# xiph/vorbis

Measured on NVIDIA H100. Metric: stereo_blocks_per_sec_mdct_psy, higher is better.
Workload: dtype f32

## Files before the change

### include/vorbis_b200.h

```cpp
#ifndef VORBIS_B200_H
#define VORBIS_B200_H

#include <stddef.h>
#include <stdint.h>

#ifdef __cplusplus
extern "C" {
#endif

#define VB200_OK        0
#define VB200_EFAULT  (-129)
#define VB200_EIMPL   (-130)
#define VB200_EINVAL  (-131)

#define VB200_P_BANDS        17
#define VB200_P_LEVELS        8
#define VB200_P_NOISECURVES   3
#define VB200_EHMER_MAX      56
#define VB200_COMPAND_LEVELS 40
#define VB200_PACKETBLOBS    15
#define VB200_MAX_CHANNELS  255
#define VB200_VE_BANDS        7
#define VB200_MAX_COUPLING  256

// ... 68 lines not shown
  float   stretch_penalty;
  float   preecho_minenergy;
  vb200_residue_setup residue[2][VB200_MAX_SUBMAPS];
} vb200_setup;

typedef struct vb200_block_desc {
  int32_t lW;
  int32_t nW;
  int32_t blocktype;
  float   ampmax;
} vb200_block_desc;

typedef struct vb200_ctx vb200_ctx;

int  vb200_ctx_create(const vb200_setup *setup, int device, vb200_ctx **out);
void vb200_ctx_destroy(vb200_ctx *ctx);
int  vb200_device_count(void);
const char *vb200_last_error(void);
int  vb200_ctx_table(vb200_ctx *ctx, int W, int which, void *dst, int cap);
uint64_t vb200_launch_count(vb200_ctx *ctx);
int  vb200_set_profiling(vb200_ctx *ctx, int on);
int  vb200_phaseA_kernel_ms(vb200_ctx *ctx, float *ms3);
int  vb200_encode_dsp_kernel_ms(vb200_ctx *ctx, float *ms6);
int  vb200_debug_phase_cycles(vb200_ctx *ctx, unsigned long long *out16, int reset);

int vb200_mdct_forward_dev (vb200_ctx*, int W, int nvec, const float *d_in, float *d_out, void *stream);
int vb200_mdct_forward     (vb200_ctx*, int W, int nvec, const float *in,   float *out);
int vb200_mdct_backward_dev(vb200_ctx*, int W, int nvec, const float *d_in, float *d_out, void *stream);
int vb200_mdct_backward    (vb200_ctx*, int W, int nvec, const float *in,   float *out);
int vb200_apply_window     (vb200_ctx*, int W, int nvec, const int32_t *lW, const int32_t *nW, float *data);
int vb200_drft_forward     (vb200_ctx*, int W, int nvec, float *data);

int vb200_noisemask        (vb200_ctx*, int look, int nvec, const float *logmdct, float *noise);
int vb200_tonemask         (vb200_ctx*, int look, int nvec, const float *logfft,
                            const float *global_specmax, const float *local_specmax, float *tone);
int vb200_offset_and_mix   (vb200_ctx*, int look, int nvec, int offset_select,
                            const float *noise, const float *tone,
                            float *mdct, const float *logmdct, float *logmask);

typedef struct vb200_phaseA_io {
  const float *pcm;
  const vb200_block_desc *desc;
  float *mdct;
  float *logmdct;
  float *logmask;
  float *ampmax_out;
  float *tap_noise;
// ... 303 lines not shown
```

### vorbis_b200/csrc/vb200.cu

```cuda
#include <cuda_runtime.h>
#include <algorithm>
#include <atomic>
#include <cstdio>
#include <cstdlib>
#include <cstring>
#include <mutex>
#include <string>
#include <type_traits>
#include <vector>

#include "vorbis_b200.h"
#include "vb200_tables.h"
#include "vb200_kernels.cuh"
#include "vb200_cqn.cuh"
#include "vb200_psy3.cuh"
#include "vb200_floor1.cuh"
#include "vb200_env.cuh"
#include "vb200_res.cuh"
#include "vb200_streams.cuh"
#include "vb200_managed.cuh"
#include "vb200_entropy_enc.cuh"
#include "vb200_bitrate.cuh"
#include "floor1_db_table.h"

// ... 405 lines not shown
  const void *src = nullptr; size_t cnt = 0, el = 4;
  switch (which) {
    case 0: src = h.trig.data(); cnt = h.trig.size(); break;
    case 1: src = h.bitrev.data(); cnt = h.bitrev.size(); break;
    case 2: src = h.win.data(); cnt = h.win.size(); break;
    case 3: src = h.wa.data(); cnt = h.wa.size(); break;
    default: return VB200_EINVAL;
  }
  if ((size_t)cap < cnt) return VB200_EINVAL;
  memcpy(dst, src, cnt * el);
  return (int)cnt;
}

extern "C" uint64_t vb200_launch_count(vb200_ctx *c) { return c ? c->launches.load() : 0; }

extern "C" int vb200_set_profiling(vb200_ctx *c, int on) {
  if (!c) return fail(VB200_EINVAL, "null context");
  CU(cudaSetDevice(c->device));
  if (on) for (auto &e : c->ev) if (!e) CU(cudaEventCreate(&e));
  c->profiling = on != 0;
  return 0;
}

extern "C" int vb200_debug_phase_cycles(vb200_ctx *c, unsigned long long *out16, int reset) {
  if (!c || !out16) return fail(VB200_EINVAL, "null argument");
  CU(cudaSetDevice(c->device));
  void *p; int rc;
  if ((rc = ensure_buf(c->cycles, 16 * sizeof(unsigned long long), &p))) return rc;
  CU(cudaDeviceSynchronize());
  CU(cudaMemcpy(out16, p, 16 * sizeof(unsigned long long), cudaMemcpyDeviceToHost));
  if (reset) CU(cudaMemset(p, 0, 16 * sizeof(unsigned long long)));
  return 0;
}

extern "C" int vb200_phaseA_kernel_ms(vb200_ctx *c, float *ms3) {
  if (!c || !ms3 || !c->ev[0]) return fail(VB200_EINVAL, "profiling not enabled");
  CU(cudaSetDevice(c->device));
  CU(cudaEventSynchronize(c->ev[3]));
  for (int i = 0; i < 3; i++) CU(cudaEventElapsedTime(ms3 + i, c->ev[i], c->ev[i + 1]));
  return 0;
}

extern "C" int vb200_encode_dsp_kernel_ms(vb200_ctx *c, float *ms6) {
  if (!c || !ms6 || !c->ev[0]) return fail(VB200_EINVAL, "profiling not enabled");
  CU(cudaSetDevice(c->device));
  CU(cudaEventSynchronize(c->ev[6]));
  for (int i = 0; i < 6; i++) CU(cudaEventElapsedTime(ms6 + i, c->ev[i], c->ev[i + 1]));
  return 0;
}


template <int NC>
__global__ void __launch_bounds__(256)
k_mdct_forward(XformDev X, int nvec, const float *__restrict__ in, float *__restrict__ out) {
  extern __shared__ __align__(16) float sm[];
  const int N = NC ? NC : X.N, tid = threadIdx.x, nt = blockDim.x;
  float *sx[2] = {sm, sm + N};
  float *sw = sm + 2 * N, *pad = sm + 3 * N;
  auto stage = [&](float *dst, int v) {
    const float *src = in + (size_t)v * N;
    const unsigned d = smem_u32(dst);
    for (int i = tid; i < (N >> 2); i += nt) cp_async16(d + 16u * (unsigned)i, src + 4 * i);
    cp_async_commit();
  };
  int v = blockIdx.x, buf = 0;
  if (v < nvec) stage(sx[0], v);
  for (; v < nvec; v += gridDim.x, buf ^= 1) {
    cp_async_wait_all();
    __syncthreads();
    if (v + (int)gridDim.x < nvec) stage(sx[buf ^ 1], v + gridDim.x);
    dev_mdct_forward<NC>(X, sx[buf], sw, out + (size_t)v * (N >> 1), tid, nt, pad);
    __syncthreads();
  }
}

template <int NC>
__global__ void __launch_bounds__(256)
k_mdct_backward(XformDev X, int nvec, const float *__restrict__ in, float *__restrict__ out) {
  extern __shared__ __align__(16) float sm[];
  const int N = NC ? NC : X.N, n2 = N >> 1, tid = threadIdx.x, nt = blockDim.x;
  float *sin_ = sm, *so = sm + n2;
  for (int v = blockIdx.x; v < nvec; v += gridDim.x) {
    const float4 *src = reinterpret_cast<const float4 *>(in + (size_t)v * n2);
    for (int i = tid; i < (n2 >> 2); i += nt) reinterpret_cast<float4 *>(sin_)[i] = __ldg(src + i);
    __syncthreads();
    dev_mdct_backward<NC>(X, sin_, so, tid, nt);
    float4 *dst = reinterpret_cast<float4 *>(out + (size_t)v * N);
    for (int i = tid; i < (N >> 2); i += nt) dst[i] = reinterpret_cast<float4 *>(so)[i];
    __syncthreads();
  }
}

__global__ void __launch_bounds__(256)
k_apply_window(WinDev Wd, int W, int nvec, const int *__restrict__ lW, const int *__restrict__ nW,
// ... 30 lines not shown
  const void *base;
  int fmt;
  int bps, hop;
  long long stride;
  const int2 *blk_src;
};

__device__ __forceinline__ void blk_origin(const PcmSrc &src, int blk, long long &st, long long &off) {
  if (src.blk_src) { const int2 o = __ldg(src.blk_src + blk); st = o.x; off = o.y; }
  else { const int s = blk / src.bps; st = s; off = (long long)(blk - s * src.bps) * src.hop; }
}

__device__ __forceinline__ float *mdct_pad_buffer(float *sf) {
#ifdef VB200_NO_FLY_PAD
  (void)sf; return nullptr;
#else
  return sf;
#endif
}

#ifndef XF_MINB
#define XF_MINB 5
#endif
template <int NC>
__global__ void __launch_bounds__(256, XF_MINB)
k_phaseA_transform(XformDev X, WinDev Wd, int W, int ch, int nrows,
                   PcmSrc src, const vb200_block_desc *__restrict__ desc,
                   float *__restrict__ mdct, float *__restrict__ logfft, float *__restrict__ lmax) {
  extern __shared__ __align__(16) float sm[];
  __shared__ float s_red[8];
  const int N = NC ? NC : X.N, n = N >> 1, tid = threadIdx.x, nt = blockDim.x;
  float *sx = sm, *sw = sm + fft_buf_floats(N), *sf = sw + N;
  const float scale = 4.f / (float)N;
  const float scale_dB = add345(todB_dev(scale));
  float *sraw = sf + fft_buf_floats(N);
  auto stage = [&](int r) -> int {
    const int b2 = r / ch, c = r - b2 * ch;
    const char *g = nullptr;
    int mode = 0;
    if (src.fmt == VB200_PCM_S16_INTERLEAVED) {
      long long st, off; blk_origin(src, b2, st, off);
      g = reinterpret_cast<const char *>(reinterpret_cast<const short *>(src.base) + (st * src.stride + off) * ch);
      mode = ch == 2 ? 2 : 0;
    } else {
      const float *pf = reinterpret_cast<const float *>(src.base);
      if (src.fmt == VB200_PCM_F32_PLANAR) {
        long long st, off; blk_origin(src, b2, st, off);
        pf += (st * ch + c) * src.stride + off;
      } else {
        pf += (size_t)r * N;
      }
      g = reinterpret_cast<const char *>(pf);
// ... 30 lines not shown
      const short *p16 = reinterpret_cast<const short *>(src.base) + (st * src.stride + off) * ch + c;
      for (int i = tid; i < N; i += nt) {
        bool z;
        const float g = dev_window_gain(Wd, W, lW, nW, i, z);
        const float v = (float)__ldg(p16 + (long long)i * ch) / 32768.f;
        sx[i] = z ? 0.f : v * g;
      }
    } else {
      const float *pf = reinterpret_cast<const float *>(src.base);
      if (src.fmt == VB200_PCM_F32_PLANAR) {
        const int c = row - blk * ch;
        long long st, off; blk_origin(src, blk, st, off);
        pf += (st * ch + c) * src.stride + off;
      } else {
        pf += (size_t)row * N;
      }
      for (int i = tid; i < N; i += nt) {
        bool z;
        const float g = dev_window_gain(Wd, W, lW, nW, i, z);
        sx[i] = z ? 0.f : __ldg(pf + i) * g;
      }
    }
    __syncthreads();
    mode = row + gridDim.x < nrows ? stage(row + gridDim.x) : 0;
    dev_mdct_forward<NC>(X, sx, sw, mdct + (size_t)row * n, tid, nt, mdct_pad_buffer(sf));
    const float *f = dev_drft_forward<NC>(X, sx, sf, tid, nt);
    float mx = -1e30f;
    float *lf = logfft + (size_t)row * n;
    for (int k = tid; k < n; k += nt) {
      float v;
      if (k == 0) {
        v = add345(scale_dB + todB_dev(f[fft_idx(0)]));
      } else {
        const float2 c = *reinterpret_cast<const float2 *>(f + fft_idx(2 * k - 1));
        const float re = c.x, im = c.y;
        const float t = re * re + im * im;
        v = add345(scale_dB + .5f * todB_dev(t));
      }
      lf[k] = v;
      mx = fmaxf(mx, v);
    }
    mx = warp_max(mx);
    if ((tid & 31) == 0) s_red[tid >> 5] = mx;
    __syncthreads();
    if (tid == 0) {
      float m = s_red[0];
      for (int w = 1; w < (nt >> 5); w++) m = fmaxf(m, s_red[w]);
      if (m > 0.f) m = 0.f;
      lmax[row] = m;
    }
    __syncthreads();
  }
}

__global__ void k_ampmax(int mode, int nstreams, int bps, int ch, const vb200_block_desc *__restrict__ desc,
                         const float *__restrict__ lmax, const float *__restrict__ amp0,
                         float secs_att, float *__restrict__ gmax) {
  const int s = blockIdx.x * blockDim.x + threadIdx.x;
  if (s >= nstreams) return;
  if (mode == 0) {
    float g = desc[s].ampmax;
    for (int c = 0; c < ch; c++) g = fmaxf(g, lmax[(size_t)s * ch + c]);
    gmax[s] = g;
    return;
  }
  float g = amp0 ? amp0[s] : -9999.f;
  float prev = g;
  for (int k = 0; k < bps; k++) {
    const size_t blk = (size_t)s * bps + k;
    if (prev > g) g = prev;
    g = g + secs_att;
    if (g < -9999.f) g = -9999.f;
    float o = g;
    for (int c = 0; c < ch; c++) o = fmaxf(o, lmax[blk * ch + c]);
// ... 469 lines not shown
  if ((rc = io.h2d(noise, bytes, &dn))) return rc;
  if ((rc = io.h2d(tone, bytes, &dt))) return rc;
  if ((rc = io.h2d(mdct, bytes, &dm))) return rc;
  if ((rc = io.h2d(logmdct, bytes, &dl))) return rc;
  if ((rc = io.h2d(nullptr, bytes, &dk))) return rc;
  k_offset_and_mix<<<grid_for(c, (int)(((size_t)nvec * P.n + 255) / 256), 8), 256, 0, c->s_main>>>(
      P, nvec, sel, (const float *)dn, (const float *)dt, (float *)dm, (const float *)dl, (float *)dk);
  if ((rc = post_launch(c))) return rc;
  if ((rc = io.d2h(logmask, dk, bytes))) return rc;
  if ((rc = io.d2h(mdct, dm, bytes))) return rc;
  return io.sync();
}

static int phaseA_transform_launch(vb200_ctx *c, int W, int nblocks, const vb200_phaseA_io *io, const PcmSrc &psrc,
                                   cudaStream_t st, float *d_logfft, float *d_lmax) {
  const XformDev &X = c->dx[W];
  const int ch = c->setup.channels, N = X.N;
  const int rows = nblocks * ch;
  {
    const size_t smem = sizeof(float) * (2 * N + 2 * fft_buf_floats(N));
    int rc;
    float *mdct_raw = io->tap_mdct_raw ? io->tap_mdct_raw : io->mdct;
    const int grid = grid_for(c, rows, 8), nt = threads_for(N);
#define LAUNCH_XF(NN)                                                                        \
    do {                                                                                     \
      if ((rc = set_smem(k_phaseA_transform<NN>, smem))) return rc;                          \
      k_phaseA_transform<NN><<<grid, nt, smem, st>>>(X, c->dwin, W, ch, rows, psrc, io->desc,    \
                                                     mdct_raw, d_logfft, d_lmax);            \
    } while (0)
    switch (N) {
      case 256: LAUNCH_XF(256); break;
      case 512: LAUNCH_XF(512); break;
      case 1024: LAUNCH_XF(1024); break;
      case 2048: LAUNCH_XF(2048); break;
      default: LAUNCH_XF(0); break;
    }
#undef LAUNCH_XF
    rc = post_launch(c); if (rc) return rc;
  }
  return 0;
}

static int phaseA_psy_launch(vb200_ctx *c, int W, int nblocks, const vb200_phaseA_io *io, cudaStream_t st,
                             float *d_logfft, float *d_lmax, float *d_gmax) {
  const int ch = c->setup.channels, n = c->dx[W].N / 2;
  const int rows = nblocks * ch;
  const PsyDev &P0 = c->dpsy[2 * W], &P1 = c->dpsy[2 * W + 1];
  const int total = P0.total > P1.total ? P0.total : P1.total;
  const int nruns = P0.nruns > P1.nruns ? P0.nruns : P1.nruns;
  const int ngrp = P0.ngrp > P1.ngrp ? P0.ngrp : P1.ngrp;
  const char *ectas = getenv("VB200_PSY_CTAS");
  const size_t smem = psy_smem_bytes(P0, P1);
  int rc = set_smem(k_phaseA_psy, smem); if (rc) return rc;
  {
    int &tuned = c->psy_carveout_ctas;
    const int ctas = ectas ? atoi(ectas) : c->psy_ctas_per_sm;
    if (tuned != ctas) {
      int pct = (int)((ctas * (smem + 1024) * 100 + 228 * 1024 - 1) / (228 * 1024));
      if (pct > 100) pct = 100;
      CU(cudaFuncSetAttribute(k_phaseA_psy, cudaFuncAttributePreferredSharedMemoryCarveout, pct));
      tuned = ctas;
    }
    c->psy_ctas_per_sm = ctas;
  }
  PsyArgs A;
  A.mdct_in = io->tap_mdct_raw ? io->tap_mdct_raw : io->mdct;
  A.logfft = d_logfft; A.lmax = d_lmax; A.gmax = d_gmax; A.desc = io->desc;
  A.mdct_out = io->mdct; A.logmdct = io->logmdct; A.logmask = io->logmask; A.ampmax_out = io->ampmax_out;
  A.tap_noise = io->tap_noise; A.tap_tone = io->tap_tone;
  A.dbg_cycles = nullptr;
  if (getenv("VB200_PHASE_TIMING")) {
    void *p; if ((rc = ensure_buf(c->cycles, 16 * sizeof(unsigned long long), &p))) return rc;
    A.dbg_cycles = (unsigned long long *)p;
  }
  const char *ev1 = getenv("VB200_PSY_V1");
  if (!(ev1 && atoi(ev1)) && P0.linesper == P1.linesper && psy3_supported(n, total, P0.linesper)) {
    constexpr int R = 2;
    const size_t row_bytes = sizeof(float) * ((psy3_floats(n, total, nruns, ngrp) + 3) & ~(size_t)3);
    const size_t smem3 = row_bytes * R;
    int ctas = (int)((227 * 1024) / (smem3 + 1024));
    if (ctas > PSY3_MINB / R) ctas = PSY3_MINB / R;
    if (ctas < 1) ctas = 1;
    if (ectas) ctas = atoi(ectas);
    const bool dbg3 = A.dbg_cycles || A.tap_noise || A.tap_tone;
#define LAUNCH_PSY3D(KK, DD)                                                                       \
    do {                                                                                           \
      if ((rc = set_smem(k_phaseA_psy3<KK, R, DD>, smem3))) return rc;                             \
      k_phaseA_psy3<KK, R, DD><<<grid_for(c, (rows + R - 1) / R, ctas), PSY3_THREADS * R, smem3, st>>>(P0, P1, ch, rows, A); \
    } while (0)
#define LAUNCH_PSY3(KK) do { if (dbg3) LAUNCH_PSY3D(KK, true); else LAUNCH_PSY3D(KK, false); } while (0)
    switch (n / 128) {
      case 1: LAUNCH_PSY3(1); break;
      case 2: LAUNCH_PSY3(2); break;
      case 4: LAUNCH_PSY3(4); break;
      case 8: LAUNCH_PSY3(8); break;
// ... 375 lines not shown
    for (int k = 0; k < ch; k++)
      if (c->setup.floor1[W][c->setup.chmux[W][k]].posts <= 0)
        return fail(VB200_EINVAL, "no floor1 setup for a channel's submap");
  }
  a->floors = c->d_floor[W]; a->chmux = c->d_chmux[W];
  a->channels = ch; a->floor_sel = floor_sel; a->nrows = nrows; a->n = c->dx[W].N / 2;
  return 0;
}

extern "C" int vb200_floor1_fit_dev(vb200_ctx *c, int W, int floor_sel, int nrows, const float *d_logmdct,
                                    const float *d_logmask, int32_t *d_posts, int32_t *d_fit_nonzero, void *stream) {
  CHECK_CTX(c); CHECK_W(W);
  if (nrows <= 0) return 0;
  Floor1Args a; int rc;
  if ((rc = floor1_args(c, W, floor_sel, nrows, &a))) return rc;
  int pcap = 2;
  for (int k = 0; k < VB200_MAX_SUBMAPS; k++) pcap = std::max(pcap, c->setup.floor1[W][k].posts);
  const size_t smem = sizeof(Floor1Dev) * VB200_MAX_SUBMAPS + floor1_fit_smem_per_warp(a.n, pcap) * F1_WARPS;
  const int ctas = (nrows + F1_WARPS - 1) / F1_WARPS;
  const bool dbg = getenv("VB200_FLOOR1_TIMING") != nullptr;
  void (*kern)(Floor1Args, int, const float *, const float *, int32_t *, int32_t *, unsigned long long *) =
      dbg ? k_floor1_fit<true> : k_floor1_fit<false>;
  void *p = nullptr;
  if (dbg && (rc = ensure_buf(c->cycles, 16 * sizeof(unsigned long long), &p))) return rc;
  if ((rc = set_smem(kern, smem))) return rc;
  CU(cudaFuncSetAttribute(kern, cudaFuncAttributePreferredSharedMemoryCarveout, cudaSharedmemCarveoutMaxShared));
  int per_sm = 0;
  CU(cudaOccupancyMaxActiveBlocksPerMultiprocessor(&per_sm, kern, 32 * F1_WARPS, smem));
  kern<<<grid_for(c, ctas, std::max(per_sm, 1)), 32 * F1_WARPS, smem, (cudaStream_t)stream>>>(
      a, pcap, d_logmdct, d_logmask, d_posts, d_fit_nonzero, (unsigned long long *)p);
  return post_launch(c);
}

static int floor1_render_launch(vb200_ctx *c, int W, int floor_sel, int nrows, int curves, long long blob_rows,
                                int32_t *d_posts, const int32_t *d_fit_nonzero, int32_t *d_ilogmask,
                                int32_t *d_nonzero, cudaStream_t st) {
  Floor1Args a; int rc;
  if ((rc = floor1_args(c, W, floor_sel, nrows, &a))) return rc;
  const int ctas = (nrows + F1_WARPS - 1) / F1_WARPS;
  k_floor1_render<<<dim3(grid_for(c, ctas, 8), curves), 32 * F1_WARPS, 0, st>>>(a, d_posts, d_fit_nonzero, d_ilogmask,
                                                                             d_nonzero, blob_rows);
  return post_launch(c);
}

extern "C" int vb200_floor1_render_dev(vb200_ctx *c, int W, int floor_sel, int nrows, int32_t *d_posts,
                                       const int32_t *d_fit_nonzero, int32_t *d_ilogmask, int32_t *d_nonzero,
                                       void *stream) {
// ... 2079 lines not shown
```

### vorbis_b200/csrc/vb200_kernels.cuh

```cuda
#pragma once
#include <cuda_runtime.h>
#include <stdint.h>
#include "vorbis_b200.h"

namespace vb200 {

#define VB_C1 .92387953251128675613F
#define VB_C2 .70710678118654752441F
#define VB_C3 .38268343236508977175F
#define VB_NEGINF (-9999.f)

struct XformDev {
  int N, log2n, nst, nf;
  int fac[8];
  int stage_off[8];
  float scale;
  const float  *trig;
  const int    *bitrev;
  const float2 *stage_tw;
  const float  *win;
  const float  *wa;
};

struct WinDev {
// ... 102 lines not shown
#pragma unroll
  for (int o = 16; o > 0; o >>= 1) v = fmaxf(v, __shfl_xor_sync(0xffffffffu, v, o));
  return v;
}


template <int NC> struct XLog2 { static constexpr int v = 1 + XLog2<NC / 2>::v; };
template <> struct XLog2<1> { static constexpr int v = 0; };
template <> struct XLog2<0> { static constexpr int v = 0; };

__device__ __forceinline__ int fly_pad(int a) { return a + 2 * (a >> 5) + 2 * (a >> 9); }

__device__ __forceinline__ void dev_fly8(const float4 v0, const float4 v1, float4 &o0, float4 &o1) {
  const float s62 = v1.z + v0.z, d62 = v1.z - v0.z;
  const float s40 = v1.x + v0.x, d40 = v1.x - v0.x;
  const float d51 = v1.y - v0.y, d73 = v1.w - v0.w;
  const float s51 = v1.y + v0.y, s73 = v1.w + v0.w;
  o1.z = s62 + s40;  o1.x = s62 - s40;
  o0.x = d62 + d51;  o0.z = d62 - d51;
  o0.w = d73 + d40;  o0.y = d73 - d40;
  o1.w = s73 + s51;  o1.y = s73 - s51;
}

template <int NC>
__device__ __forceinline__ void dev_butterflies(const XformDev &X, float *x, int tid, int nt, float *padbuf = nullptr) {
  const int N = NC ? NC : X.N;
  const int log2n = NC ? XLog2<NC>::v : X.log2n;
  const int nst = log2n - 6;
  const int n2 = N >> 1;
  const int items = n2 >> 2;
#pragma unroll
  for (int s = 0; s < nst; s++) {
    const int P = n2 >> s;
    const int lq = P >> 2;
    const int sh = log2n - 3 - s;
    const float2 *tw = X.stage_tw + X.stage_off[s];
    for (int u = tid; u < items; u += nt) {
      const int blk = u >> sh, q = u & (lq - 1);
      float *xb = x + P * blk;
      const int a = P - 2 - 2 * q, b = (P >> 1) - 2 - 2 * q;
      const float2 t = __ldg(tw + q);
      const float2 hi = *reinterpret_cast<float2 *>(xb + a);
      const float2 lo = *reinterpret_cast<float2 *>(xb + b);
      const float r0 = hi.x - lo.x, r1 = hi.y - lo.y;
      *reinterpret_cast<float2 *>(xb + a) = make_float2(hi.x + lo.x, hi.y + lo.y);
      *reinterpret_cast<float2 *>(xb + b) = make_float2(r1 * t.y + r0 * t.x, r1 * t.x - r0 * t.y);
// ... 46 lines not shown
    }
    {
      const float o0 = v3.z - v1.z, o1 = v3.w - v1.w;
      v3.z = v3.z + v1.z; v3.w = v3.w + v1.w;
      v1.z = o0; v1.w = o1;
    }
    float4 o0, o1, o2, o3;
    dev_fly8(v0, v1, o0, o1);
    dev_fly8(v2, v3, o2, o3);
    if (padbuf) {
      float2 *q = reinterpret_cast<float2 *>(padbuf + fly_pad(16 * u));
      q[0] = make_float2(o0.x, o0.y); q[1] = make_float2(o0.z, o0.w);
      q[2] = make_float2(o1.x, o1.y); q[3] = make_float2(o1.z, o1.w);
      float2 *r = reinterpret_cast<float2 *>(padbuf + fly_pad(16 * u + 8));
      r[0] = make_float2(o2.x, o2.y); r[1] = make_float2(o2.z, o2.w);
      r[2] = make_float2(o3.x, o3.y); r[3] = make_float2(o3.z, o3.w);
    } else {
      p[0] = o0; p[1] = o1; p[2] = o2; p[3] = o3;
    }
  }
  __syncthreads();
}

template <int NC>
__device__ __forceinline__ void dev_bitreverse(const XformDev &X, float *w, int tid, int nt, const float *padbuf = nullptr) {
  const int N = NC ? NC : X.N, n2 = N >> 1;
  const float2 *T = reinterpret_cast<const float2 *>(X.trig + N);
  const int2 *br = reinterpret_cast<const int2 *>(X.bitrev);
  const float *x = w + n2;
  for (int m = tid; m < (N >> 3); m += nt) {
    const int2 b = __ldg(br + m);
    const float2 t = __ldg(T + m);
    const float2 x0 = padbuf ? *reinterpret_cast<const float2 *>(padbuf + fly_pad(b.x)) : *reinterpret_cast<const float2 *>(x + b.x);
    const float2 x1 = padbuf ? *reinterpret_cast<const float2 *>(padbuf + fly_pad(b.y)) : *reinterpret_cast<const float2 *>(x + b.y);
    const float r0 = x0.y - x1.y;
    const float r1 = x0.x + x1.x;
    const float r2 = r1 * t.x + r0 * t.y;
    const float r3 = r1 * t.y - r0 * t.x;
    const float h0 = (x0.y + x1.y) * .5f;
    const float h1 = (x0.x - x1.x) * .5f;
    *reinterpret_cast<float2 *>(w + 2 * m) = make_float2(h0 + r2, h1 + r3);
    *reinterpret_cast<float2 *>(w + n2 - 2 * m - 2) = make_float2(h0 - r2, r3 - h1);
  }
  __syncthreads();
}

template <int NC>
__device__ __forceinline__ void dev_mdct_forward(const XformDev &X, const float *in, float *w,
                                                 float *out, int tid, int nt, float *padbuf = nullptr) {
  const int N = NC ? NC : X.N, n2 = N >> 1, n4 = N >> 2, n16 = N >> 4;
  float *w2 = w + n2;
  const float2 *Tf = reinterpret_cast<const float2 *>(X.trig);
  for (int p = tid; p < n4; p += nt) {
    const float2 t = __ldg(Tf + (n4 - 1 - p));
    float r0, r1;
    if (p < n16) {
      const float4 a = *reinterpret_cast<const float4 *>(in + n2 + n4 - 4 * (p + 1));
      const float4 b = *reinterpret_cast<const float4 *>(in + n2 + n4 + 4 * p);
      r0 = a.z + b.y;
      r1 = a.x + b.w;
    } else if (p < n4 - n16) {
      const float4 a = *reinterpret_cast<const float4 *>(in + n2 + n4 - 4 * (p + 1));
      const float4 b = *reinterpret_cast<const float4 *>(in + 4 * (p - n16));
      r0 = a.z - b.y;
      r1 = a.x - b.w;
    } else {
      const float4 a = *reinterpret_cast<const float4 *>(in + N - 4 * (p - (n4 - n16) + 1));
      const float4 b = *reinterpret_cast<const float4 *>(in + 4 * (p - n16));
      r0 = -a.z - b.y;
      r1 = -a.x - b.w;
    }
    *reinterpret_cast<float2 *>(w2 + 2 * p) = make_float2(r1 * t.y + r0 * t.x, r1 * t.x - r0 * t.y);
  }
  __syncthreads();
  dev_butterflies<NC>(X, w2, tid, nt, padbuf);
  dev_bitreverse<NC>(X, w, tid, nt, padbuf);
  const float2 *Tp = reinterpret_cast<const float2 *>(X.trig + n2);
  const float scale = X.scale;
  for (int i = tid; i < n4; i += nt) {
    const float2 v = *reinterpret_cast<const float2 *>(w + 2 * i);
    const float2 t = __ldg(Tp + i);
    out[i]          = (v.x * t.x + v.y * t.y) * scale;
    out[n2 - 1 - i] = (v.x * t.y - v.y * t.x) * scale;
  }
}

template <int NC>
__device__ __forceinline__ void dev_mdct_backward(const XformDev &X, const float *in, float *out,
                                                  int tid, int nt) {
  const int N = NC ? NC : X.N, n2 = N >> 1, n4 = N >> 2, n16 = N >> 4;
  const float *T = X.trig;
  for (int u = tid; u < 2 * n16; u += nt) {
    if (u < n16) {
      const int j = u;
      const float *iX = in + n2 - 7 - 8 * j;
      const float4 t = __ldg(reinterpret_cast<const float4 *>(T + n4 + 4 * j));
      float4 o;
      o.x = -iX[2] * t.w - iX[0] * t.z;
      o.y =  iX[0] * t.w - iX[2] * t.z;
      o.z = -iX[6] * t.y - iX[4] * t.x;
      o.w =  iX[4] * t.y - iX[6] * t.x;
      *reinterpret_cast<float4 *>(out + n2 + n4 - 4 * (j + 1)) = o;
    } else {
      const int j = u - n16;
      const float *iX = in + n2 - 8 - 8 * j;
      const float4 t = __ldg(reinterpret_cast<const float4 *>(T + n4 - 4 * (j + 1)));
      float4 o;
// ... 139 lines not shown
    const int o = 2 * k * ido;
    if (ii == 0) {
      const float a0 = cc[fft_rd<FIRST>(c0)], a1 = cc[fft_rd<FIRST>(c1)];
      ch[fft_idx(o)]               = a0 + a1;
      ch[fft_idx(o + 2 * ido - 1)] = a0 - a1;
      *reinterpret_cast<float2 *>(ch + fft_idx(o + ido - 1)) =
          make_float2(cc[fft_rd<FIRST>(c0 + ido - 1)], -cc[fft_rd<FIRST>(c1 + ido - 1)]);
    } else {
      const int i = 2 * ii;
      const float wr = __ldg(w1 + i - 2), wi = __ldg(w1 + i - 1);
      const int r0 = fft_rd<FIRST>(c0 + i - 1);
      const int r1 = FIRST ? r0 + t0 : ((t0 & 31) == 0 ? r0 + t0 + (t0 >> 4) : fft_idx(c1 + i - 1));
      const float2 a0 = *reinterpret_cast<const float2 *>(cc + r0);
      const float2 a1 = *reinterpret_cast<const float2 *>(cc + r1);
      const float tr2 = wr * a1.x + wi * a1.y;
      const float ti2 = wr * a1.y - wi * a1.x;
      const int ic = 2 * ido - i;
      *reinterpret_cast<float2 *>(ch + fft_idx(o + i - 1))  = make_float2(a0.x + tr2, a0.y + ti2);
      *reinterpret_cast<float2 *>(ch + fft_idx(o + ic - 1)) = make_float2(a0.x - tr2, ti2 - a0.y);
    }
  }
}

template <int NC>
__device__ __forceinline__ float *dev_drft_forward(const XformDev &X, float *a, float *b,
                                                   int tid, int nt) {
  const int N = NC ? NC : X.N;
  const int log2n = NC ? XLog2<NC>::v : X.log2n;
  const int nf = (log2n + 1) >> 1;
  int l2 = N, iw = N;
  float *src = a, *dst = b;
#pragma unroll
  for (int k1 = 0; k1 < nf; k1++) {
    const int ip = (k1 == nf - 1 && (log2n & 1)) ? 2 : 4;
    const int l1 = l2 / ip, ido = N / l2;
    iw -= (ip - 1) * ido;
    if (k1 == 0) {
      if (ip == 4) dev_fft_pass4<true>(ido, l1, src, dst, X.wa + iw - 1, X.wa + iw + ido - 1, X.wa + iw + 2 * ido - 1, tid, nt);
      else dev_fft_pass2<true>(ido, l1, src, dst, X.wa + iw - 1, tid, nt);
    } else {
      if (ip == 4) dev_fft_pass4<false>(ido, l1, src, dst, X.wa + iw - 1, X.wa + iw + ido - 1, X.wa + iw + 2 * ido - 1, tid, nt);
      else dev_fft_pass2<false>(ido, l1, src, dst, X.wa + iw - 1, tid, nt);
    }
    __syncthreads();
    float *t = src; src = dst; dst = t;
    l2 = l1;
  }
  return src;
}

__device__ __forceinline__ float dev_window_gain(const WinDev &Wd, int W, int lW, int nW, int i,
                                                 bool &zero) {
  if (!W) { lW = 0; nW = 0; }
  const int n = Wd.N[W], ln = Wd.N[lW], rn = Wd.N[nW];
  const int leftbegin = n / 4 - ln / 4, leftend = leftbegin + ln / 2;
  const int rightbegin = n / 2 + n / 4 - rn / 4, rightend = rightbegin + rn / 2;
  zero = false;
  if (i < leftbegin || i >= rightend) { zero = true; return 0.f; }
  if (i < leftend) return __ldg(Wd.win[lW] + (i - leftbegin));
  if (i >= rightbegin) return __ldg(Wd.win[nW] + (rn / 2 - 1 - (i - rightbegin)));
  return 1.f;
}

__device__ __forceinline__ float4 dev_window4(const WinDev &Wd, int W, int lW, int nW, int i0, float4 x) {
  if (!W) { lW = 0; nW = 0; }
  const int n = Wd.N[W], ln = Wd.N[lW], rn = Wd.N[nW];
  const int leftbegin = n / 4 - ln / 4, leftend = leftbegin + ln / 2;
// ... 407 lines not shown
```

### vorbis_b200/lib.py

```python
import ctypes as C
import os

import numpy as np

from . import abi

HERE = os.path.dirname(os.path.abspath(__file__))
LIB_PATH = os.path.join(HERE, "libvorbis_b200.so")

PCM_F32_PLANAR = 1
PCM_S16_INTERLEAVED = 2
IWORK_S32 = 0
IWORK_S16 = 1

EXPORTS = [
    "vb200_ctx_create", "vb200_ctx_destroy", "vb200_device_count", "vb200_last_error",
    "vb200_ctx_table", "vb200_launch_count", "vb200_set_profiling", "vb200_phaseA_kernel_ms", "vb200_debug_phase_cycles",
    "vb200_encode_dsp_kernel_ms",
    "vb200_mdct_forward_dev", "vb200_mdct_forward", "vb200_mdct_backward_dev", "vb200_mdct_backward",
    "vb200_apply_window", "vb200_drft_forward",
    "vb200_noisemask", "vb200_tonemask", "vb200_offset_and_mix",
    "vb200_analysis_phaseA_dev", "vb200_analysis_phaseA", "vb200_analysis_phaseA_streams_dev",
    "vb200_analysis_phaseA_pcmstream_dev", "vb200_synthesis_s16_dev",
    "vb200_couple_quantize_normalize_dev", "vb200_couple_quantize_normalize",
    "vb200_synthesis_dev", "vb200_synthesis", "vb200_synthesis_halfrate", "vb200_decouple_dev", "vb200_decouple",
    "vb200_floor1_fit_dev", "vb200_floor1_fit", "vb200_floor1_render_dev", "vb200_floor1_render",
    "vb200_encode_dsp_dev", "vb200_encode_dsp", "vb200_encode_dsp_managed_dev", "vb200_encode_dsp_managed",
    "vb200_envelope_search_dev", "vb200_envelope_search", "vb200_envelope_search_var", "vb200_envelope_apply_marks",
    "vb200_floor1_inverse2_dev", "vb200_floor1_inverse2", "vb200_decode_dsp_dev", "vb200_decode_dsp",
    "vb200_decode_dsp_resume_dev", "vb200_decode_dsp_resume",
    "vb200_decode_entropy_setup", "vb200_decode_entropy_dev", "vb200_decode_entropy",
    "vb200_decode_packets_resume_dev", "vb200_decode_packets_resume",
    "vb200_encode_entropy_setup", "vb200_encode_packet_bound", "vb200_encode_entropy_dev", "vb200_encode_entropy",
    "vb200_encode_packets", "vb200_encode_entropy_managed_dev", "vb200_encode_packets_managed",
    "vb200_residue_partvals", "vb200_residue_classify_dev", "vb200_residue_classify",
    "vb200_plan_blocks", "vb200_encode_streams_dev", "vb200_encode_streams",
# ... 12 lines not shown


class VB200Error(RuntimeError):
    pass


_lib = None


def load():
    global _lib
    if _lib is not None:
        return _lib
    if not os.path.exists(LIB_PATH):
        raise VB200Error("%s not found: build it with `python -c 'import __graft_entry__ as g; g.build()'`"
                         % LIB_PATH)
    L = C.CDLL(LIB_PATH)
    L.vb200_last_error.restype = C.c_char_p
    L.vb200_launch_count.restype = C.c_uint64
    L.vb200_launch_count.argtypes = [vp]
    L.vb200_set_profiling.argtypes = [vp, C.c_int]
    L.vb200_phaseA_kernel_ms.argtypes = [vp, C.POINTER(C.c_float * 3)]
    L.vb200_encode_dsp_kernel_ms.argtypes = [vp, C.POINTER(C.c_float * 6)]
    L.vb200_debug_phase_cycles.argtypes = [vp, C.POINTER(C.c_ulonglong * 16), C.c_int]
    L.vb200_ctx_create.argtypes = [C.POINTER(abi.Setup), C.c_int, C.POINTER(vp)]
    L.vb200_ctx_destroy.argtypes = [vp]
    L.vb200_ctx_table.argtypes = [vp, C.c_int, C.c_int, vp, C.c_int]
    L.vb200_mdct_forward_dev.argtypes = [vp, C.c_int, C.c_int, vp, vp, vp]
    L.vb200_mdct_backward_dev.argtypes = [vp, C.c_int, C.c_int, vp, vp, vp]
    L.vb200_mdct_forward.argtypes = [vp, C.c_int, C.c_int, vp, vp]
    L.vb200_mdct_backward.argtypes = [vp, C.c_int, C.c_int, vp, vp]
    L.vb200_apply_window.argtypes = [vp, C.c_int, C.c_int, vp, vp, f32p]
    L.vb200_drft_forward.argtypes = [vp, C.c_int, C.c_int, f32p]
    L.vb200_noisemask.argtypes = [vp, C.c_int, C.c_int, f32p, f32p]
    L.vb200_tonemask.argtypes = [vp, C.c_int, C.c_int, f32p, f32p, f32p, f32p]
    L.vb200_offset_and_mix.argtypes = [vp, C.c_int, C.c_int, C.c_int, f32p, f32p, f32p, f32p, f32p]
    L.vb200_analysis_phaseA_dev.argtypes = [vp, C.c_int, C.c_int, C.POINTER(abi.PhaseAIO), vp]
    L.vb200_analysis_phaseA.argtypes = [vp, C.c_int, C.c_int, C.POINTER(abi.PhaseAIO)]
    L.vb200_analysis_phaseA_streams_dev.argtypes = [vp, C.c_int, C.c_int, C.c_int, C.POINTER(abi.PhaseAIO), vp, vp]
    L.vb200_analysis_phaseA_pcmstream_dev.argtypes = [vp, C.c_int, C.c_int, C.c_int, vp, C.c_int, C.c_int64, C.c_int,
                                                      C.POINTER(abi.PhaseAIO), vp, vp]
    L.vb200_synthesis_s16_dev.argtypes = [vp, C.c_int, C.c_int, vp, vp, vp, vp, vp, C.c_int64, vp]
    L.vb200_couple_quantize_normalize_dev.argtypes = [vp, C.c_int, C.c_int, C.c_int, C.c_int, vp, vp, vp, vp]
    L.vb200_couple_quantize_normalize.argtypes = [vp, C.c_int, C.c_int, C.c_int, C.c_int, vp, vp, vp]
    L.vb200_synthesis_dev.argtypes = [vp, C.c_int, C.c_int, vp, vp, vp, vp, vp, C.c_int64, vp]
    L.vb200_synthesis.argtypes = [vp, C.c_int, C.c_int, vp, vp, vp, C.c_int64, vp, vp, C.c_int64]
    L.vb200_synthesis_halfrate.argtypes = [vp, C.c_int, vp]
# ... 107 lines not shown
    def __del__(self):
        try:
            self.close()
        except Exception:
            pass

    def launch_count(self):
        return int(self.L.vb200_launch_count(self.h))

    def set_profiling(self, on=True):
        self._chk(self.L.vb200_set_profiling(self.h, 1 if on else 0))

    def phaseA_kernel_ms(self):
        ms = (C.c_float * 3)()
        self._chk(self.L.vb200_phaseA_kernel_ms(self.h, C.byref(ms)))
        return [float(x) for x in ms]

    def encode_dsp_kernel_ms(self):
        ms = (C.c_float * 6)()
        self._chk(self.L.vb200_encode_dsp_kernel_ms(self.h, C.byref(ms)))
        return list(ms)

    def debug_phase_cycles(self, reset=True):
        out = (C.c_ulonglong * 16)()
        self._chk(self.L.vb200_debug_phase_cycles(self.h, C.byref(out), 1 if reset else 0))
        return [int(x) for x in out]

    def table(self, W, which):
        N = self.bs[W]
        out = np.zeros(N // 4, np.int32) if which == 1 else np.zeros(2 * N, np.float32)
        k = self.L.vb200_ctx_table(self.h, W, which, out.ctypes.data, out.size)
        if k <= 0:
            raise VB200Error("vb200_ctx_table failed")
        return out[:k].copy()

    def mdct_forward(self, W, x):
        x = np.ascontiguousarray(x, np.float32).reshape(-1, self.bs[W])
        out = np.empty((x.shape[0], self.bs[W] // 2), np.float32)
        self._chk(self.L.vb200_mdct_forward(self.h, W, x.shape[0], _ptr(x), _ptr(out)))
        return out

    def mdct_backward(self, W, x):
        N = self.bs[W] >> self.halfrate
        x = np.ascontiguousarray(x, np.float32).reshape(-1, N // 2)
        out = np.empty((x.shape[0], N), np.float32)
        self._chk(self.L.vb200_mdct_backward(self.h, W, x.shape[0], _ptr(x), _ptr(out)))
        return out
# ... 682 lines not shown
```

Baseline: 5.715 million.

## Restructure MDCT butterflies into radix-4 blocked stages with fused prerotation and bitreverse

Adds a blocked butterfly path for the forward MDCT. Pairs of radix-2 stages are merged into one pass per sync, the pre-rotation is fused into the first stage when the stage count allows, the final 32- and 16-point butterflies are specialised, and bit-reversal is fused with post-rotation. Both the standalone and phase-A transform kernels now use it, and a trailing __syncthreads is dropped from the phase-A row loop. The aim is fewer shared-memory round trips and barriers per row, at the cost of more register pressure and new indexing that could be wrong. It also adds optional clock64 timing marks selected by an environment variable and widens the debug slot buffer.

```diff
diff --git a/include/vorbis_b200.h b/include/vorbis_b200.h
--- a/include/vorbis_b200.h
+++ b/include/vorbis_b200.h
@@ -114,7 +114,8 @@
 int  vb200_set_profiling(vb200_ctx *ctx, int on);
 int  vb200_phaseA_kernel_ms(vb200_ctx *ctx, float *ms3);
 int  vb200_encode_dsp_kernel_ms(vb200_ctx *ctx, float *ms6);
-int  vb200_debug_phase_cycles(vb200_ctx *ctx, unsigned long long *out16, int reset);
+#define VB200_DEBUG_SLOTS 32
+int  vb200_debug_phase_cycles(vb200_ctx *ctx, unsigned long long *out, int reset);
 
 int vb200_mdct_forward_dev (vb200_ctx*, int W, int nvec, const float *d_in, float *d_out, void *stream);
 int vb200_mdct_forward     (vb200_ctx*, int W, int nvec, const float *in,   float *out);
diff --git a/vorbis_b200/csrc/vb200.cu b/vorbis_b200/csrc/vb200.cu
--- a/vorbis_b200/csrc/vb200.cu
+++ b/vorbis_b200/csrc/vb200.cu
@@ -451,14 +451,14 @@
   return 0;
 }
 
-extern "C" int vb200_debug_phase_cycles(vb200_ctx *c, unsigned long long *out16, int reset) {
-  if (!c || !out16) return fail(VB200_EINVAL, "null argument");
+extern "C" int vb200_debug_phase_cycles(vb200_ctx *c, unsigned long long *out, int reset) {
+  if (!c || !out) return fail(VB200_EINVAL, "null argument");
   CU(cudaSetDevice(c->device));
   void *p; int rc;
-  if ((rc = ensure_buf(c->cycles, 16 * sizeof(unsigned long long), &p))) return rc;
+  if ((rc = ensure_buf(c->cycles, VB200_DEBUG_SLOTS * sizeof(unsigned long long), &p))) return rc;
   CU(cudaDeviceSynchronize());
-  CU(cudaMemcpy(out16, p, 16 * sizeof(unsigned long long), cudaMemcpyDeviceToHost));
-  if (reset) CU(cudaMemset(p, 0, 16 * sizeof(unsigned long long)));
+  CU(cudaMemcpy(out, p, VB200_DEBUG_SLOTS * sizeof(unsigned long long), cudaMemcpyDeviceToHost));
+  if (reset) CU(cudaMemset(p, 0, VB200_DEBUG_SLOTS * sizeof(unsigned long long)));
   return 0;
 }
 
@@ -498,7 +498,7 @@
     cp_async_wait_all();
     __syncthreads();
     if (v + (int)gridDim.x < nvec) stage(sx[buf ^ 1], v + gridDim.x);
-    dev_mdct_forward<NC>(X, sx[buf], sw, out + (size_t)v * (N >> 1), tid, nt, pad);
+    dev_mdct_forward<NC, true>(X, sx[buf], sw, out + (size_t)v * (N >> 1), tid, nt, pad);
     __syncthreads();
   }
 }
@@ -575,12 +575,14 @@
 #ifndef XF_MINB
 #define XF_MINB 5
 #endif
-template <int NC>
+template <int NC, bool DBG>
 __global__ void __launch_bounds__(256, XF_MINB)
 k_phaseA_transform(XformDev X, WinDev Wd, int W, int ch, int nrows,
                    PcmSrc src, const vb200_block_desc *__restrict__ desc,
-                   float *__restrict__ mdct, float *__restrict__ logfft, float *__restrict__ lmax) {
+                   float *__restrict__ mdct, float *__restrict__ logfft, float *__restrict__ lmax,
+                   unsigned long long *dbg) {
   extern __shared__ __align__(16) float sm[];
+  XfMarks<DBG> mk{dbg, DBG ? clock64() : 0};
   __shared__ float s_red[8];
   const int N = NC ? NC : X.N, n = N >> 1, tid = threadIdx.x, nt = blockDim.x;
   float *sx = sm, *sw = sm + fft_buf_floats(N), *sf = sw + N;
@@ -657,9 +659,10 @@
       }
     }
     __syncthreads();
+    if (DBG) mk(XF_T_WINDOW);
     mode = row + gridDim.x < nrows ? stage(row + gridDim.x) : 0;
-    dev_mdct_forward<NC>(X, sx, sw, mdct + (size_t)row * n, tid, nt, mdct_pad_buffer(sf));
-    const float *f = dev_drft_forward<NC>(X, sx, sf, tid, nt);
+    dev_mdct_forward<NC, true, DBG>(X, sx, sw, mdct + (size_t)row * n, tid, nt, mdct_pad_buffer(sf), &mk);
+    const float *f = dev_drft_forward<NC, DBG>(X, sx, sf, tid, nt, &mk);
     float mx = -1e30f;
     float *lf = logfft + (size_t)row * n;
     for (int k = tid; k < n; k += nt) {
@@ -678,13 +681,13 @@
     mx = warp_max(mx);
     if ((tid & 31) == 0) s_red[tid >> 5] = mx;
     __syncthreads();
+    if (DBG) { mk(XF_T_LOG); if (tid == 0) atomicAdd(dbg + XF_T_ROWS, 1ull); }
     if (tid == 0) {
       float m = s_red[0];
       for (int w = 1; w < (nt >> 5); w++) m = fmaxf(m, s_red[w]);
       if (m > 0.f) m = 0.f;
       lmax[row] = m;
     }
-    __syncthreads();
   }
 }
 
@@ -1200,11 +1203,15 @@
     int rc;
     float *mdct_raw = io->tap_mdct_raw ? io->tap_mdct_raw : io->mdct;
     const int grid = grid_for(c, rows, 8), nt = threads_for(N);
-#define LAUNCH_XF(NN)                                                                        \
-    do {                                                                                     \
-      if ((rc = set_smem(k_phaseA_transform<NN>, smem))) return rc;                          \
-      k_phaseA_transform<NN><<<grid, nt, smem, st>>>(X, c->dwin, W, ch, rows, psrc, io->desc,    \
-                                                     mdct_raw, d_logfft, d_lmax);            \
+    const bool dbg = getenv("VB200_XFORM_TIMING") != nullptr;
+    void *p = nullptr;
+    if (dbg && (rc = ensure_buf(c->cycles, VB200_DEBUG_SLOTS * sizeof(unsigned long long), &p))) return rc;
+#define LAUNCH_XF(NN)                                                                              \
+    do {                                                                                           \
+      auto kern = dbg ? k_phaseA_transform<NN, true> : k_phaseA_transform<NN, false>;             \
+      if ((rc = set_smem(kern, smem))) return rc;                                                  \
+      kern<<<grid, nt, smem, st>>>(X, c->dwin, W, ch, rows, psrc, io->desc, mdct_raw, d_logfft,    \
+                                   d_lmax, (unsigned long long *)p);                               \
     } while (0)
     switch (N) {
       case 256: LAUNCH_XF(256); break;
@@ -1248,7 +1255,7 @@
   A.tap_noise = io->tap_noise; A.tap_tone = io->tap_tone;
   A.dbg_cycles = nullptr;
   if (getenv("VB200_PHASE_TIMING")) {
-    void *p; if ((rc = ensure_buf(c->cycles, 16 * sizeof(unsigned long long), &p))) return rc;
+    void *p; if ((rc = ensure_buf(c->cycles, VB200_DEBUG_SLOTS * sizeof(unsigned long long), &p))) return rc;
     A.dbg_cycles = (unsigned long long *)p;
   }
   const char *ev1 = getenv("VB200_PSY_V1");
@@ -1670,7 +1677,7 @@
   void (*kern)(Floor1Args, int, const float *, const float *, int32_t *, int32_t *, unsigned long long *) =
       dbg ? k_floor1_fit<true> : k_floor1_fit<false>;
   void *p = nullptr;
-  if (dbg && (rc = ensure_buf(c->cycles, 16 * sizeof(unsigned long long), &p))) return rc;
+  if (dbg && (rc = ensure_buf(c->cycles, VB200_DEBUG_SLOTS * sizeof(unsigned long long), &p))) return rc;
   if ((rc = set_smem(kern, smem))) return rc;
   CU(cudaFuncSetAttribute(kern, cudaFuncAttributePreferredSharedMemoryCarveout, cudaSharedmemCarveoutMaxShared));
   int per_sm = 0;
diff --git a/vorbis_b200/csrc/vb200_kernels.cuh b/vorbis_b200/csrc/vb200_kernels.cuh
--- a/vorbis_b200/csrc/vb200_kernels.cuh
+++ b/vorbis_b200/csrc/vb200_kernels.cuh
@@ -148,6 +148,69 @@
   o1.w = s73 + s51;  o1.y = s73 - s51;
 }
 
+__device__ __forceinline__ void dev_r2(float2 &hi, float2 &lo, const float2 t) {
+  const float r0 = hi.x - lo.x, r1 = hi.y - lo.y;
+  hi = make_float2(hi.x + lo.x, hi.y + lo.y);
+  lo = make_float2(r1 * t.y + r0 * t.x, r1 * t.x - r0 * t.y);
+}
+
+__device__ __forceinline__ void dev_fly32(float2 &hi, float2 &lo, int q) {
+  const float dxp = hi.x - lo.x, dxn = lo.x - hi.x, dyp = hi.y - lo.y, dyn = lo.y - hi.y;
+  const float r0 = q >= 5 ? dxn : dxp;
+  const float r1 = q >= 4 ? dyn : dyp;
+  const bool q15 = (q == 1) | (q == 7);
+  const float k00 = q15 ? VB_C1 : VB_C3;
+  const float k3 = q15 ? VB_C3 : VB_C1;
+  const float k01 = q < 4 ? -k3 : k3;
+  const float k10 = q < 4 ? k3 : -k3;
+  const float A0 = r0 * k00 + r1 * k01;
+  const float A1 = r0 * k10 + r1 * k00;
+  const float B0 = (q == 2 ? r0 - r1 : r1 + r0) * VB_C2;
+  const float B1 = (q == 2 ? r0 + r1 : r1 - r0) * VB_C2;
+  const float T0 = q == 0 ? r0 : r1, T1 = q == 0 ? r1 : r0;
+  const bool odd = q & 1, triv = (q & 3) == 0;
+  hi = make_float2(hi.x + lo.x, hi.y + lo.y);
+  lo = make_float2(odd ? A0 : (triv ? T0 : B0), odd ? A1 : (triv ? T1 : B1));
+}
+
+__device__ __forceinline__ void dev_fly16(float *x, int u, float *padbuf) {
+  float4 *p = reinterpret_cast<float4 *>(x + 16 * u);
+  float4 v0 = p[0], v1 = p[1], v2 = p[2], v3 = p[3];
+  {
+    const float a = v0.y - v2.y, b = v0.x - v2.x;
+    v2.x = v2.x + v0.x; v2.y = v2.y + v0.y;
+    v0.x = (a + b) * VB_C2; v0.y = (a - b) * VB_C2;
+  }
+  {
+    const float o0 = v0.w - v2.w, o1 = v2.z - v0.z;
+    v2.z = v2.z + v0.z; v2.w = v2.w + v0.w;
+    v0.z = o0; v0.w = o1;
+  }
+  {
+    const float a = v3.x - v1.x, b = v3.y - v1.y;
+    v3.x = v3.x + v1.x; v3.y = v3.y + v1.y;
+    v1.x = (a - b) * VB_C2; v1.y = (a + b) * VB_C2;
+  }
+  {
+    const float o0 = v3.z - v1.z, o1 = v3.w - v1.w;
+    v3.z = v3.z + v1.z; v3.w = v3.w + v1.w;
+    v1.z = o0; v1.w = o1;
+  }
+  float4 o0, o1, o2, o3;
+  dev_fly8(v0, v1, o0, o1);
+  dev_fly8(v2, v3, o2, o3);
+  if (padbuf) {
+    float2 *q = reinterpret_cast<float2 *>(padbuf + fly_pad(16 * u));
+    q[0] = make_float2(o0.x, o0.y); q[1] = make_float2(o0.z, o0.w);
+    q[2] = make_float2(o1.x, o1.y); q[3] = make_float2(o1.z, o1.w);
+    float2 *r = reinterpret_cast<float2 *>(padbuf + fly_pad(16 * u + 8));
+    r[0] = make_float2(o2.x, o2.y); r[1] = make_float2(o2.z, o2.w);
+    r[2] = make_float2(o3.x, o3.y); r[3] = make_float2(o3.z, o3.w);
+  } else {
+    p[0] = o0; p[1] = o1; p[2] = o2; p[3] = o3;
+  }
+}
+
 template <int NC>
 __device__ __forceinline__ void dev_butterflies(const XformDev &X, float *x, int tid, int nt, float *padbuf = nullptr) {
   const int N = NC ? NC : X.N;
@@ -240,6 +303,126 @@
   __syncthreads();
 }
 
+enum { XF_T_WINDOW, XF_T_PREROT, XF_T_STAGE, XF_T_FLY32 = XF_T_STAGE + 7, XF_T_FLY16, XF_T_BITREV, XF_T_POSTROT,
+       XF_T_FFT, XF_T_LOG = XF_T_FFT + 7, XF_T_ROWS, XF_T_SLOTS };
+template <bool DBG> struct XfMarks {
+  unsigned long long *dbg;
+  long long t;
+  __device__ __forceinline__ void operator()(int slot) {
+    if (DBG && threadIdx.x == 0) {
+      const long long u = clock64();
+      atomicAdd(dbg + slot, (unsigned long long)(u - t));
+      t = u;
+    }
+  }
+  __device__ __forceinline__ void cut(int slot) { if (DBG) { __syncthreads(); (*this)(slot); } }
+};
+
+template <int NC>
+__device__ __forceinline__ float2 dev_mdct_prerot(const XformDev &X, const float *in, int p) {
+  const int N = NC ? NC : X.N, n2 = N >> 1, n4 = N >> 2, n16 = N >> 4;
+  const float2 t = __ldg(reinterpret_cast<const float2 *>(X.trig) + (n4 - 1 - p));
+  float r0, r1;
+  if (p < n16) {
+    const float4 a = *reinterpret_cast<const float4 *>(in + n2 + n4 - 4 * (p + 1));
+    const float4 b = *reinterpret_cast<const float4 *>(in + n2 + n4 + 4 * p);
+    r0 = a.z + b.y;
+    r1 = a.x + b.w;
+  } else if (p < n4 - n16) {
+    const float4 a = *reinterpret_cast<const float4 *>(in + n2 + n4 - 4 * (p + 1));
+    const float4 b = *reinterpret_cast<const float4 *>(in + 4 * (p - n16));
+    r0 = a.z - b.y;
+    r1 = a.x - b.w;
+  } else {
+    const float4 a = *reinterpret_cast<const float4 *>(in + N - 4 * (p - (n4 - n16) + 1));
+    const float4 b = *reinterpret_cast<const float4 *>(in + 4 * (p - n16));
+    r0 = -a.z - b.y;
+    r1 = -a.x - b.w;
+  }
+  return make_float2(r1 * t.y + r0 * t.x, r1 * t.x - r0 * t.y);
+}
+
+template <int NC, bool DBG>
+__device__ __forceinline__ void dev_butterflies_blocked(const XformDev &X, float *x, int tid, int nt, float *padbuf,
+                                                        XfMarks<DBG> *mk, const float *pre_in = nullptr) {
+  const int N = NC ? NC : X.N;
+  const int log2n = NC ? XLog2<NC>::v : X.log2n;
+  const int nst = log2n - 6;
+  const int n2 = N >> 1;
+  const int groups = n2 >> 3;
+  int s = 0;
+  if (nst > 0 && (nst & 1) == 0) {
+    const float2 *tw = X.stage_tw;
+    for (int u = tid; u < (n2 >> 2); u += nt) {
+      float2 hi = *reinterpret_cast<float2 *>(x + n2 - 2 - 2 * u), lo = *reinterpret_cast<float2 *>(x + (n2 >> 1) - 2 - 2 * u);
+      dev_r2(hi, lo, __ldg(tw + u));
+      *reinterpret_cast<float2 *>(x + n2 - 2 - 2 * u) = hi;
+      *reinterpret_cast<float2 *>(x + (n2 >> 1) - 2 - 2 * u) = lo;
+    }
+    __syncthreads();
+    if (DBG) (*mk)(XF_T_STAGE);
+    s = 1;
+  }
+#pragma unroll
+  for (; s + 1 < nst; s += 2) {
+    const int P = n2 >> s;
+    const int lq = P >> 3;
+    const int sh = log2n - 4 - s;
+    const float2 *t0 = X.stage_tw + X.stage_off[s], *t1 = X.stage_tw + X.stage_off[s + 1];
+    for (int g = tid; g < groups; g += nt) {
+      const int q = g & (lq - 1);
+      float *xb = x + P * (g >> sh) - 2 - 2 * q;
+      float2 *pa = reinterpret_cast<float2 *>(xb + P), *pb = reinterpret_cast<float2 *>(xb + 3 * (P >> 2));
+      float2 *pc = reinterpret_cast<float2 *>(xb + (P >> 1)), *pd = reinterpret_cast<float2 *>(xb + (P >> 2));
+      float2 a, b, c, d;
+      if (s == 0 && pre_in) {
+        a = dev_mdct_prerot<NC>(X, pre_in, (N >> 2) - 1 - q);
+        b = dev_mdct_prerot<NC>(X, pre_in, 3 * (N >> 4) - 1 - q);
+        c = dev_mdct_prerot<NC>(X, pre_in, (N >> 3) - 1 - q);
+        d = dev_mdct_prerot<NC>(X, pre_in, (N >> 4) - 1 - q);
+      } else {
+        a = *pa; b = *pb; c = *pc; d = *pd;
+      }
+      dev_r2(a, c, __ldg(t0 + q));
+      dev_r2(b, d, __ldg(t0 + q + lq));
+      const float2 u = __ldg(t1 + q);
+      dev_r2(a, b, u);
+      dev_r2(c, d, u);
+      *pa = a; *pb = b; *pc = c; *pd = d;
+    }
+    __syncthreads();
+    if (DBG) (*mk)(XF_T_STAGE + s);
+  }
+  if (nst > 0) {
+    const float2 *t0 = X.stage_tw + X.stage_off[nst - 1];
+    for (int g = tid; g < groups; g += nt) {
+      const int q = g & 7;
+      float *xb = x + 64 * (g >> 3) - 2 * q;
+      float2 *pa = reinterpret_cast<float2 *>(xb + 62), *pb = reinterpret_cast<float2 *>(xb + 46);
+      float2 *pc = reinterpret_cast<float2 *>(xb + 30), *pd = reinterpret_cast<float2 *>(xb + 14);
+      float2 a = *pa, b = *pb, c = *pc, d = *pd;
+      dev_r2(a, c, __ldg(t0 + q));
+      dev_r2(b, d, __ldg(t0 + q + 8));
+      dev_fly32(a, b, q);
+      dev_fly32(c, d, q);
+      *pa = a; *pb = b; *pc = c; *pd = d;
+    }
+  } else {
+    for (int u = tid; u < (n2 >> 2); u += nt) {
+      float *xc = x + 32 * (u >> 3);
+      const int q = u & 7;
+      float2 hi = *reinterpret_cast<float2 *>(xc + 30 - 2 * q), lo = *reinterpret_cast<float2 *>(xc + 14 - 2 * q);
+      dev_fly32(hi, lo, q);
+      *reinterpret_cast<float2 *>(xc + 30 - 2 * q) = hi;
+      *reinterpret_cast<float2 *>(xc + 14 - 2 * q) = lo;
+    }
+  }
+  __syncthreads();
+  if (DBG) (*mk)(XF_T_FLY32);
+  for (int u = tid; u < (n2 >> 4); u += nt) dev_fly16(x, u, padbuf);
+  __syncthreads();
+}
+
 template <int NC>
 __device__ __forceinline__ void dev_bitreverse(const XformDev &X, float *w, int tid, int nt, const float *padbuf = nullptr) {
   const int N = NC ? NC : X.N, n2 = N >> 1;
@@ -264,35 +447,58 @@
 }
 
 template <int NC>
+__device__ __forceinline__ void dev_bitreverse_rotate(const XformDev &X, const float *x, float *out, int tid, int nt,
+                                                      const float *padbuf) {
+  const int N = NC ? NC : X.N, n2 = N >> 1, n4 = N >> 2;
+  const float2 *T = reinterpret_cast<const float2 *>(X.trig + N);
+  const float2 *Tp = reinterpret_cast<const float2 *>(X.trig + n2);
+  const int2 *br = reinterpret_cast<const int2 *>(X.bitrev);
+  const float scale = X.scale;
+  for (int m = tid; m < (N >> 3); m += nt) {
+    const int2 b = __ldg(br + m);
+    const float2 t = __ldg(T + m);
+    const float2 x0 = padbuf ? *reinterpret_cast<const float2 *>(padbuf + fly_pad(b.x)) : *reinterpret_cast<const float2 *>(x + b.x);
+    const float2 x1 = padbuf ? *reinterpret_cast<const float2 *>(padbuf + fly_pad(b.y)) : *reinterpret_cast<const float2 *>(x + b.y);
+    const float r0 = x0.y - x1.y;
+    const float r1 = x0.x + x1.x;
+    const float r2 = r1 * t.x + r0 * t.y;
+    const float r3 = r1 * t.y - r0 * t.x;
+    const float h0 = (x0.y + x1.y) * .5f;
+    const float h1 = (x0.x - x1.x) * .5f;
+    const float2 v0 = make_float2(h0 + r2, h1 + r3), v1 = make_float2(h0 - r2, r3 - h1);
+    const int i = n4 - 1 - m;
+    const float2 ta = __ldg(Tp + m), tb = __ldg(Tp + i);
+    out[m]          = (v0.x * ta.x + v0.y * ta.y) * scale;
+    out[n2 - 1 - m] = (v0.x * ta.y - v0.y * ta.x) * scale;
+    out[i]          = (v1.x * tb.x + v1.y * tb.y) * scale;
+    out[n2 - 1 - i] = (v1.x * tb.y - v1.y * tb.x) * scale;
+  }
+  __syncthreads();
+}
+
+template <int NC, bool BLOCKED = false, bool DBG = false>
 __device__ __forceinline__ void dev_mdct_forward(const XformDev &X, const float *in, float *w,
-                                                 float *out, int tid, int nt, float *padbuf = nullptr) {
-  const int N = NC ? NC : X.N, n2 = N >> 1, n4 = N >> 2, n16 = N >> 4;
+                                                 float *out, int tid, int nt, float *padbuf = nullptr,
+                                                 XfMarks<DBG> *mk = nullptr) {
+  const int N = NC ? NC : X.N, n2 = N >> 1, n4 = N >> 2;
+  const int nst = (NC ? XLog2<NC>::v : X.log2n) - 6;
   float *w2 = w + n2;
-  const float2 *Tf = reinterpret_cast<const float2 *>(X.trig);
-  for (int p = tid; p < n4; p += nt) {
-    const float2 t = __ldg(Tf + (n4 - 1 - p));
-    float r0, r1;
-    if (p < n16) {
-      const float4 a = *reinterpret_cast<const float4 *>(in + n2 + n4 - 4 * (p + 1));
-      const float4 b = *reinterpret_cast<const float4 *>(in + n2 + n4 + 4 * p);
-      r0 = a.z + b.y;
-      r1 = a.x + b.w;
-    } else if (p < n4 - n16) {
-      const float4 a = *reinterpret_cast<const float4 *>(in + n2 + n4 - 4 * (p + 1));
-      const float4 b = *reinterpret_cast<const float4 *>(in + 4 * (p - n16));
-      r0 = a.z - b.y;
-      r1 = a.x - b.w;
-    } else {
-      const float4 a = *reinterpret_cast<const float4 *>(in + N - 4 * (p - (n4 - n16) + 1));
-      const float4 b = *reinterpret_cast<const float4 *>(in + 4 * (p - n16));
-      r0 = -a.z - b.y;
-      r1 = -a.x - b.w;
-    }
-    *reinterpret_cast<float2 *>(w2 + 2 * p) = make_float2(r1 * t.y + r0 * t.x, r1 * t.x - r0 * t.y);
-  }
-  __syncthreads();
-  dev_butterflies<NC>(X, w2, tid, nt, padbuf);
+  const bool fuse_pre = BLOCKED && nst >= 3 && (nst & 1);
+  if (!fuse_pre) {
+    for (int p = tid; p < n4; p += nt) *reinterpret_cast<float2 *>(w2 + 2 * p) = dev_mdct_prerot<NC>(X, in, p);
+    __syncthreads();
+    if (DBG) (*mk)(XF_T_PREROT);
+  }
+  if (BLOCKED) dev_butterflies_blocked<NC, DBG>(X, w2, tid, nt, padbuf, mk, fuse_pre ? in : nullptr);
+  else dev_butterflies<NC>(X, w2, tid, nt, padbuf);
+  if (DBG) (*mk)(XF_T_FLY16);
+  if (BLOCKED) {
+    dev_bitreverse_rotate<NC>(X, w2, out, tid, nt, padbuf);
+    if (DBG) (*mk)(XF_T_BITREV);
+    return;
+  }
   dev_bitreverse<NC>(X, w, tid, nt, padbuf);
+  if (DBG) (*mk)(XF_T_BITREV);
   const float2 *Tp = reinterpret_cast<const float2 *>(X.trig + n2);
   const float scale = X.scale;
   for (int i = tid; i < n4; i += nt) {
@@ -301,6 +507,7 @@
     out[i]          = (v.x * t.x + v.y * t.y) * scale;
     out[n2 - 1 - i] = (v.x * t.y - v.y * t.x) * scale;
   }
+  if (DBG) mk->cut(XF_T_POSTROT);
 }
 
 template <int NC>
@@ -486,9 +693,9 @@
   }
 }
 
-template <int NC>
+template <int NC, bool DBG = false>
 __device__ __forceinline__ float *dev_drft_forward(const XformDev &X, float *a, float *b,
-                                                   int tid, int nt) {
+                                                   int tid, int nt, XfMarks<DBG> *mk = nullptr) {
   const int N = NC ? NC : X.N;
   const int log2n = NC ? XLog2<NC>::v : X.log2n;
   const int nf = (log2n + 1) >> 1;
@@ -507,6 +714,7 @@
       else dev_fft_pass2<false>(ido, l1, src, dst, X.wa + iw - 1, tid, nt);
     }
     __syncthreads();
+    if (DBG) (*mk)(XF_T_FFT + k1);
     float *t = src; src = dst; dst = t;
     l2 = l1;
   }
diff --git a/vorbis_b200/lib.py b/vorbis_b200/lib.py
--- a/vorbis_b200/lib.py
+++ b/vorbis_b200/lib.py
@@ -12,6 +12,7 @@
 PCM_S16_INTERLEAVED = 2
 IWORK_S32 = 0
 IWORK_S16 = 1
+DEBUG_SLOTS = 32
 
 EXPORTS = [
     "vb200_ctx_create", "vb200_ctx_destroy", "vb200_device_count", "vb200_last_error",
@@ -70,7 +71,7 @@
     L.vb200_set_profiling.argtypes = [vp, C.c_int]
     L.vb200_phaseA_kernel_ms.argtypes = [vp, C.POINTER(C.c_float * 3)]
     L.vb200_encode_dsp_kernel_ms.argtypes = [vp, C.POINTER(C.c_float * 6)]
-    L.vb200_debug_phase_cycles.argtypes = [vp, C.POINTER(C.c_ulonglong * 16), C.c_int]
+    L.vb200_debug_phase_cycles.argtypes = [vp, C.POINTER(C.c_ulonglong * DEBUG_SLOTS), C.c_int]
     L.vb200_ctx_create.argtypes = [C.POINTER(abi.Setup), C.c_int, C.POINTER(vp)]
     L.vb200_ctx_destroy.argtypes = [vp]
     L.vb200_ctx_table.argtypes = [vp, C.c_int, C.c_int, vp, C.c_int]
@@ -224,7 +225,7 @@
         return list(ms)
 
     def debug_phase_cycles(self, reset=True):
-        out = (C.c_ulonglong * 16)()
+        out = (C.c_ulonglong * DEBUG_SLOTS)()
         self._chk(self.L.vb200_debug_phase_cycles(self.h, C.byref(out), 1 if reset else 0))
         return [int(x) for x in out]
 
```

After: 5.859 million, median of 6. 2.5% higher.
